# Xiuyu-Li/q-diffusion

Measured on AMD Instinct MI355X. Metric: denoising images/sec (whole node), SD-v1.4 W4A8 512x512 50-step PLMS, higher is better.
Workload: dtype int8xint4->int32 (fp32 residual stream); 1 GPU; sd UNet eval batch 16 per GPU, 51 evals per image batch, W4A8 sm_abit=16 split, hip-graph=on, cross-attention K/V of the run's context prepared once per image batch (2.82 ms, charged as /51 per step); images_per_gpu=8, global_batch=8, context_prepared=True, parallelism=batch-sharded x1, quant-state broadcast 0 B

## Files before the change

q-diffusion_amd/csrc/igemm_dma.hip:

```cpp
#include "common.h"
#include <type_traits>

typedef __attribute__((address_space(3))) void* qd_lds_ptr;

namespace {

__device__ __attribute__((aligned(16))) const int qd_zero16[4] = {0, 0, 0, 0};

struct SegD {
    int c0, clen, kstep0, nsteps_tap;
    const float*  scale;
    const int*    zc;
    const int*    zw;
    const int*    zfill;
    const int8_t* fill16;
};

struct ConvD {
    const int8_t*  x;
    const uint8_t* wt;
    void*          out;
    int32_t*       iout;
    const float*   bias;
    const float*   rowbias;
    const void*    residual;
    long ldx, ldo, ldr, ldrb;
    int B, H, W, Ho, Wo, Cout, kh, kw, stride, pad_t, pad_l;
    int M, taps, nseg, nblk_m, nblk_n, ntiles;
    int vec;
    SegD seg[2];
    const float* oq;
    float oqmin, oqmax;
    int   oqoff;
    int   it_per;
    int   hdH, hdd, hdT, hdTpad, hddpad;
    unsigned hdrcp;
    float oqpre;
    int32_t* hdsum;
    float* gnpart;
    int    gn_nchunk;
    long   gn_ld;
    int    pointwise;
    int    res_f16;
    int    res_period;
    int    ups;
};

enum { O_F32 = 0, O_F16 = 1, O_I32 = 2, O_GEGLU = 3, O_PART = 4, O_HROWS = 5, O_HTR = 6, O_BF16 = 7, O_GEGLU_H = 8 };

template <int N>
__device__ __forceinline__ void wait_vmcnt() {
    asm volatile("s_waitcnt vmcnt(%0)" ::"n"(N) : "memory");
}

__device__ __forceinline__ void glds16(const void* gsrc, unsigned lds_base) {
#ifdef QD_ABL_NODMA
    asm volatile("" ::"v"(gsrc), "s"(lds_base) : "memory");
    return;
#endif
    asm volatile(
        "s_mov_b32 m0, %1\n\t"
        "s_nop 0\n\t"
        "global_load_lds_dwordx4 %0, off"
        :
        : "v"(gsrc), "s"(lds_base)
        : "memory");
}

__device__ __forceinline__ int bytesum16(const v4i& v) {
    int s = __builtin_amdgcn_sdot4(v.x, 0x01010101, 0, false);
    s = __builtin_amdgcn_sdot4(v.y, 0x01010101, s, false);
    s = __builtin_amdgcn_sdot4(v.z, 0x01010101, s, false);
    return __builtin_amdgcn_sdot4(v.w, 0x01010101, s, false);
}

__device__ __forceinline__ unsigned lds_addr(const void* p) {
    return (unsigned)(size_t)(qd_lds_ptr)(p);
}

__device__ __forceinline__ constexpr int crow(int r) { return (r & 3) + 8 * (r >> 2); }

#ifndef QD_MT1_OCC
#define QD_MT1_OCC 2
#endif
template <int MT, int NT, int WM, int WN, int OUT, int WB, int KS = 1>
__host__ __device__ constexpr int igemm_smem_bytes() {
    constexpr bool BF = WB >= 16;
    constexpr int BM = 32 * MT * WM, BN = 32 * NT * WN, NTB = NT * WN;
    constexpr int TB = BF ? 2048 : 256 * WB;
    constexpr int STAGE = BM * 64 + NTB * TB;
    constexpr int TBW = ((OUT == O_F16 || OUT == O_HROWS) && !BF) ? 8192 : 4096;
    constexpr int EPI_BYTES = 4 * KS * TBW + 4 * (32 * NT) * 8;
    constexpr int RING = 3 * KS * STAGE > EPI_BYTES ? 3 * KS * STAGE : EPI_BYTES;
    return RING + (2 + (KS > 1 ? 1 : 0)) * BM * 4 + 4 * BN * 4;
}

template <int MT, int NT, int WM, int WN, bool SPLIT, int OUT, int WB, int KS = 1>
__device__ __forceinline__ void igemm_body(const ConvD& p, unsigned char* smem) {
    static_assert(KS == 1 || (KS == 2 && !SPLIT && WB <= 8 && (OUT == O_F32 || OUT == O_F16 || OUT == O_PART || OUT == O_HROWS || OUT == O_HTR)),
                  "two K-groups: one segment; linear rows, split-K partials or the head-layout epilogues");
    static_assert(WB == 4 || WB == 8 || WB == 16 || WB == 17, "weight bits (16 = bf16 mode, 17 = fp16 mode)");
    constexpr bool BF = WB >= 16;
    constexpr bool FH = WB == 17;
    static_assert(!BF || (!SPLIT && (OUT == O_F32 || OUT == (FH ? O_F16 : O_BF16))), "16-bit float mode: one segment, fp32 rows or rows of the operand type");
    static_assert(WM * WN == 4, "four waves per block");
    constexpr int BM = 32 * MT * WM, BN = 32 * NT * WN, NTB = NT * WN;
    constexpr int TB = BF ? 2048 : 256 * WB;
    constexpr int A_BYTES = BM * 64, B_BYTES = NTB * TB;
    constexpr int STAGE = A_BYTES + B_BYTES;
    constexpr int NA = BM / 64;
    constexpr int NBI = B_BYTES / 1024;
    constexpr int NBW = (NBI + 3) / 4;
    constexpr int PER = NA + NBW;
    constexpr int WCOLS = 32 * NT;

    constexpr int TBW = ((OUT == O_F16 || OUT == O_HROWS) && !BF) ? 8192 : 4096;
    constexpr int EPI_BYTES = 4 * KS * TBW + 4 * WCOLS * 8;
    constexpr int RS = KS * STAGE;
    constexpr int RING = 3 * RS > EPI_BYTES ? 3 * RS : EPI_BYTES;
    static_assert(RING + (2 + (KS > 1 ? 1 : 0)) * BM * 4 + 4 * BN * 4 == igemm_smem_bytes<MT, NT, WM, WN, OUT, WB, KS>(), "igemm_smem_bytes out of step with the body");
    int* sRowB = reinterpret_cast<int*>(smem + RING);
    int* sAsum = sRowB + BM;
    int* sAsum1 = sAsum + BM;
    float* sScale = reinterpret_cast<float*>(sAsum + (KS > 1 ? 2 : 1) * BM);
    int*   sZc    = reinterpret_cast<int*>(sScale + BN);
    int*   sZw    = sZc + BN;
    float* sBias  = reinterpret_cast<float*>(sZw + BN);

    const int lane = threadIdx.x & 63;
    const int wave_all = __builtin_amdgcn_readfirstlane(threadIdx.x >> 6);
    const int kg = KS > 1 ? wave_all >> 2 : 0;
    const int wave = wave_all & 3;
    const int wm = wave / WN, wn = wave % WN;
    const int frow = lane & 31, fhalf = lane >> 5;

    const int nblk    = p.nblk_m * p.nblk_n;
    const int logical = qd_xcd_remap(blockIdx.x, nblk);
    const int mb = logical / p.nblk_n, nb = logical % p.nblk_n;
    const int m0 = mb * BM, n0 = nb * BN;

    const int lr16 = lane >> 2, slot = lane & 3;
    const int a_chunk = (slot ^ ((lr16 >> 2) & 3)) * 16;
    const int8_t* a_org[NA];
    unsigned a_mask[NA];
    int a_hw0[NA];
    bool a_valid[NA];
    const int HoWo = p.Ho * p.Wo;
    if (p.pointwise) {
#pragma unroll
        for (int i = 0; i < NA; ++i) {
            const int r = (wave + 4 * i) * 16 + lr16;
            const int m = m0 + r;
            a_valid[i] = m < p.M;
            const int mm = a_valid[i] ? m : 0;
            a_org[i] = p.x + (long)mm * p.ldx + a_chunk;
            a_mask[i] = a_valid[i] ? 1u : 0u;
            a_hw0[i] = 0;
            if (p.rowbias != nullptr && slot == 0) sRowB[r] = mm / HoWo;
        }
    } else {
#pragma unroll
    for (int i = 0; i < NA; ++i) {
        const int r = (wave + 4 * i) * 16 + lr16;
// ... 819 lines not shown
            int as[16];
            row_terms(rbase, as);
#pragma unroll
            for (int r = 0; r < 16; ++r) {
                const int rl = crow(r) + 4 * fhalf;
                const int I0 = acc[i][j][r] - zc0 - __mul24(zw0, as[r]);
                const int I1 = acc[i][j + 1][r] - zc1 - __mul24(zw1, as[r]);
                float v0, v1;
                if (SPLIT) {
                    v0 = __builtin_fmaf((float)I0, sc0, facc[SPLIT ? i : 0][SPLIT ? j : 0][r]) + bias0;
                    v1 = __builtin_fmaf((float)I1, sc1, facc[SPLIT ? i : 0][SPLIT ? j + 1 : 0][r]) + bias1;
                } else {
                    v0 = __builtin_fmaf((float)I0, sc0, bias0);
                    v1 = __builtin_fmaf((float)I1, sc1, bias1);
                }
                if (rb_tile) { v0 += rbv0; v1 += rbv1; }
                const int pc = frow ^ ((r & 1) << 2);
                tb[rl * 64 + pc] = __float_as_uint(v0);
                tb[rl * 64 + 32 + pc] = __float_as_uint(v1);
            }
            __builtin_amdgcn_sched_barrier(0);
#pragma unroll
            for (int pb = 0; pb < 4; pb += 2) {
            v4i rs[2];
            long mrow[2];
#pragma unroll
            for (int u = 0; u < 2; ++u) {
                const long m = m0 + rbase + (pb + u) * 8 + rr0;
                mrow[u] = m < p.M ? m : m0;
                if (has_res) rs[u] = *reinterpret_cast<const v4i*>(rh + res_row(mrow[u]) * p.ldr + n8c);
            }
#pragma unroll
            for (int u = 0; u < 2; ++u) {
                const int rl = (pb + u) * 8 + rr0;
                const bool mok = m0 + rbase + rl < p.M;
                v4f lo = *reinterpret_cast<const v4f*>(tb + rl * 64 + rd_lo);
                v4f hi = *reinterpret_cast<const v4f*>(tb + rl * 64 + rd_hi);
                if (has_rb && !rb_tile) {
                    const float* src = p.rowbias + (long)sRowB[rbase + rl] * p.ldrb + n8c;
                    lo += *reinterpret_cast<const v4f*>(src);
                    hi += *reinterpret_cast<const v4f*>(src + 4);
                }
                if (has_res) {
                    v4f a, b;
                    qd_h8_to_f(rs[u], a, b);
                    lo += a; hi += b;
                }
                if (mok && nok8) {
                    const v4i pk = {(int)qd_pack2h(lo[0], lo[1]), (int)qd_pack2h(lo[2], lo[3]),
                                    (int)qd_pack2h(hi[0], hi[1]), (int)qd_pack2h(hi[2], hi[3])};
                    *reinterpret_cast<v4i*>(oh + mrow[u] * p.ldo + n8) = pk;
                    if (gn) {
#pragma unroll
                        for (int e = 0; e < 4; ++e) {
                            gs[e] += lo[e]; gq[e] = __builtin_fmaf(lo[e], lo[e], gq[e]);
                            gs[4 + e] += hi[e]; gq[4 + e] = __builtin_fmaf(hi[e], hi[e], gq[4 + e]);
                        }
                    }
                }
            }
            }
        }
        if (gn) {
#pragma unroll
            for (int e = 0; e < 8; ++e) {
#pragma unroll
                for (int sh = 8; sh < 64; sh <<= 1) {
                    gs[e] += __shfl_xor(gs[e], sh);
                    gq[e] += __shfl_xor(gq[e], sh);
                }
            }
            if (lane < 8) {
#pragma unroll
                for (int e = 0; e < 8; ++e) {
                    sGn[(wave * WCOLS + j * 32 + k8 * 8 + e) * 2] = gs[e];
                    sGn[(wave * WCOLS + j * 32 + k8 * 8 + e) * 2 + 1] = gq[e];
                }
            }
        }
        }
    };
    bool lines16 = false;
    if constexpr (H16_OUT && !BF) lines16 = p.vec == 2;
    if (lines16) {
#pragma unroll
        for (int q = 0; q < NT / 2; ++q)
            if (owner(2 * q) == kg) pair(2 * q);
        if constexpr (NT % 2 == 1) {
            if (owner(NT - 1) == kg) single(NT - 1);
        }
    } else {
#pragma unroll
        for (int j = 0; j < NT; ++j)
            if (owner(j) == kg) single(j);
    }
    if (gn) {
        __syncthreads();
        for (int c = threadIdx.x; c < BN; c += 256 * KS)
        if (n0 + c < p.Cout) {
            constexpr int WPC = MT >= 4 ? 1 : 4 / MT;
            const int wnc = c / WCOLS, cw = c - wnc * WCOLS;
#pragma unroll
            for (int ch = 0; ch < BM / 128; ++ch) {
                const int mrow = m0 + ch * 128;
                if (mrow >= p.M) break;
                float ts = 0.f, tq = 0.f;
#pragma unroll
                for (int w = 0; w < WPC; ++w) {
                    const int wv = (ch * WPC + w) * WN + wnc;
                    ts += sGn[(wv * WCOLS + cw) * 2];
                    tq += sGn[(wv * WCOLS + cw) * 2 + 1];
                }
                const int b = mrow / HoWo, chunk = (mrow - b * HoWo) >> 7;
                float* dst = p.gnpart + (((long)b * p.gn_nchunk + chunk) * p.gn_ld + n0 + c) * 2;
                dst[0] = ts;
                dst[1] = tq;
            }
        }
    }
}

template <int MT, int NT, int WM, int WN, bool SPLIT, int OUT, int WB>
__global__ __launch_bounds__(256, (SPLIT || MT * NT > 10) ? 1 : (MT == 1 && NT <= 5 ? QD_MT1_OCC : 2)) void igemm_kernel(const ConvD p) {
    __shared__ __attribute__((aligned(16))) unsigned char smem[igemm_smem_bytes<MT, NT, WM, WN, OUT, WB>()];
    igemm_body<MT, NT, WM, WN, SPLIT, OUT, WB>(p, smem);
}

template <int MT, int NT, int WM, int WN, int OUT, int WB>
__global__ __launch_bounds__(512, 1) void igemm_k2_kernel(const ConvD p) {
    __shared__ __attribute__((aligned(16))) unsigned char smem[igemm_smem_bytes<MT, NT, WM, WN, OUT, WB, 2>()];
    igemm_body<MT, NT, WM, WN, false, OUT, WB, 2>(p, smem);
}

struct ConvG {
    ConvD d[3];
    int   out[3];
};
template <int MT, int NT, int WM, int WN, int WB>
__global__ __launch_bounds__(256, (MT * NT > 10) ? 1 : (MT == 1 && NT <= 5 ? QD_MT1_OCC : 2)) void igemm_heads_group_kernel(const ConvG g) {
    constexpr int SA = igemm_smem_bytes<MT, NT, WM, WN, O_HROWS, WB>(), SB = igemm_smem_bytes<MT, NT, WM, WN, O_HTR, WB>();
    __shared__ __attribute__((aligned(16))) unsigned char smem[SA > SB ? SA : SB];
    const int z = blockIdx.y;
    if (g.out[z] == O_HTR) igemm_body<MT, NT, WM, WN, false, O_HTR, WB>(g.d[z], smem);
    else igemm_body<MT, NT, WM, WN, false, O_HROWS, WB>(g.d[z], smem);
}

__global__ __launch_bounds__(256) void pack_t4_kernel(const float* __restrict__ w, const float* __restrict__ alpha,
                                                      const float* __restrict__ delta, const float* __restrict__ zp,
                                                      int Cout, int Cin_total, int taps, int c0, int clen, int clen_pad,
                                                      int n_levels, uint8_t* __restrict__ wt, int kstep0, int ntiles,
                                                      int nsteps_tap, int32_t* __restrict__ wsum) {
    long gid = (long)blockIdx.x * 256 + threadIdx.x;
    const long total = (long)taps * nsteps_tap * ntiles * 128;
    if (gid >= total) return;
    const int nn = (int)(gid & 31);
    const int kh4 = (int)((gid >> 5) & 3);
    long rest = gid >> 7;
    const int jt = (int)(rest % ntiles);
    rest /= ntiles;
    const int cs = (int)(rest % nsteps_tap);
    const int t = (int)(rest / nsteps_tap);
    const int n = jt * 32 + nn;
    const int cbase = cs * 64 + kh4 * 16;
    int vals[16];
    int sum = 0;
    float d = 1.f, z = 0.f;
    if (n < Cout) { d = delta[n]; z = zp[n]; }
// ... 23 lines not shown
    *reinterpret_cast<uint2*>(wt + (kstep * ntiles + jt) * 1024 + (kh4 * 32 + nn) * 8) = pk;
    if (wsum && sum != 0) atomicAdd(&wsum[n], sum);
}

template <typename TO>
__global__ __launch_bounds__(256) void splitk_finalize_kernel(const int32_t* __restrict__ part, int nsplit, long MN, int Cout, int HoWo,
                                                              const float* __restrict__ scale, const int* __restrict__ zc,
                                                              const int* __restrict__ zw, const int* __restrict__ zfill,
                                                              const float* __restrict__ bias, const float* __restrict__ rowbias, long ldrb,
                                                              const TO* __restrict__ residual, long ldr, TO* __restrict__ out, long ldo) {
    const long e = (long)blockIdx.x * 256 + threadIdx.x;
    if (e >= MN) return;
    const long m = e / Cout;
    const int  n = (int)(e - m * Cout);
    int I = 0;
    for (int s = 0; s < nsplit; ++s) I += part[(long)s * MN + e];
    const int kz = zfill ? zfill[1] : 0;
    I = I - (zc ? zc[n] : 0) + (zw ? zw[n] : 0) * kz;
    float v = __builtin_fmaf((float)I, scale[n], bias ? bias[n] : 0.f);
    if (rowbias) v += rowbias[(m / HoWo) * ldrb + n];
    if constexpr (std::is_same<TO, float>::value) {
        if (residual) v += residual[m * ldr + n];
        out[m * ldo + n] = v;
    } else {
        if (residual) v += __half2float(residual[m * ldr + n]);
        out[m * ldo + n] = __float2half(v);
    }
}

__global__ __launch_bounds__(256) void pack_t8_kernel(const float* __restrict__ w, const float* __restrict__ alpha,
                                                      const float* __restrict__ delta, const float* __restrict__ zp,
                                                      int Cout, int Cin_total, int taps, int c0, int clen,
                                                      int n_levels, uint8_t* __restrict__ wt, int kstep0, int ntiles,
                                                      int nsteps_tap, int32_t* __restrict__ wsum) {
    long gid = (long)blockIdx.x * 256 + threadIdx.x;
    const long total = (long)taps * nsteps_tap * ntiles * 128;
    if (gid >= total) return;
    const int nn = (int)(gid & 31);
    const int kh4 = (int)((gid >> 5) & 3);
    long rest = gid >> 7;
    const int jt = (int)(rest % ntiles);
    rest /= ntiles;
    const int cs = (int)(rest % nsteps_tap);
    const int t = (int)(rest / nsteps_tap);
    const int n = jt * 32 + nn;
    const int cbase = cs * 64 + kh4 * 16;
    int sum = 0;
    float d = 1.f, z = 0.f;
    if (n < Cout) { d = delta[n]; z = zp[n]; }
    v4i pk;
#pragma unroll
    for (int g = 0; g < 4; ++g) {
        unsigned word = 0;
#pragma unroll
        for (int e = 0; e < 4; ++e) {
            const int c = cbase + g * 4 + e;
            int stored = 0;
            if (n < Cout && c < clen) {
                const float wv = w[((long)n * Cin_total + c0 + c) * taps + t];
                float q;
                if (alpha) q = floorf(wv / d) + (alpha[((long)n * clen + c) * taps + t] >= 0.f ? 1.f : 0.f);
                else q = rintf(wv / d);
                q = fminf(fmaxf(q + z, 0.f), (float)(n_levels - 1));
                stored = (int)q - 128;
                sum += stored;
            }
            word |= (unsigned)(stored & 0xff) << (8 * e);
        }
        pk[g] = (int)word;
    }
    const long kstep = kstep0 + (long)t * nsteps_tap + cs;
    *reinterpret_cast<v4i*>(wt + (kstep * ntiles + jt) * 2048 + (kh4 * 32 + nn) * 16) = pk;
    if (wsum && sum != 0) atomicAdd(&wsum[n], sum);
}

#ifdef QD_PROBE_INSTANCE
template __global__ void igemm_kernel<QD_PROBE_INSTANCE>(const ConvD);
}
#else
static int& kgroups_knob() {
    static int v = (getenv("QD_KGROUPS") && atoi(getenv("QD_KGROUPS")) == 0) ? 0 : 1;
    return v;
}

constexpr int kgroups_min_steps() { return 8; }

struct TileId {
    int mt, nt, wm, wn, wb;
    constexpr int bm() const { return 32 * mt * wm; }
    constexpr int bn() const { return 32 * nt * wn; }
    constexpr bool operator==(const TileId& o) const { return mt == o.mt && nt == o.nt && wm == o.wm && wn == o.wn && wb == o.wb; }
};
template <int MT, int NT, int WM, int WN, int WB>
struct Tile { static constexpr TileId id{MT, NT, WM, WN, WB}; };
template <class F>
bool visit_tile(const TileId& id, F f) {
    auto among = [&](auto... t) { return ((decltype(t)::id == id && (f(t), true)) || ...); };
    return among(Tile<1, 5, 4, 1, 4>{}, Tile<1, 7, 4, 1, 4>{}, Tile<1, 4, 4, 1, 4>{}, Tile<1, 2, 4, 1, 4>{}, Tile<2, 5, 4, 1, 4>{}, Tile<2, 4, 4, 1, 4>{}, Tile<2, 5, 2, 2, 4>{},
                 Tile<1, 4, 4, 1, 8>{}, Tile<1, 2, 4, 1, 8>{}, Tile<2, 4, 4, 1, 8>{}, Tile<1, 4, 4, 1, 16>{}, Tile<1, 2, 4, 1, 16>{}, Tile<2, 4, 4, 1, 16>{},
                 Tile<1, 4, 4, 1, 17>{}, Tile<1, 2, 4, 1, 17>{}, Tile<2, 4, 4, 1, 17>{});
}

template <class T>
constexpr bool built(int KS, bool SPLIT, int OUT) {
    constexpr int MT = T::id.mt, NT = T::id.nt, WM = T::id.wm, WB = T::id.wb;
    constexpr bool rows128 = MT == 1 && WM == 4;
    const bool rows = OUT == O_F32 || OUT == O_F16, heads = OUT == O_HROWS || OUT == O_HTR;
    if (WB >= 16) return KS == 1 && !SPLIT && (OUT == O_F32 || OUT == (WB == 16 ? O_BF16 : O_F16));
    if (KS == 2)
        return !SPLIT && (WM == 4 || (MT == 2 && NT == 5)) && (NT == 4 || NT == 5 || NT == 7) && (WB == 4 || NT == 4) &&
               (OUT == O_F32 || (OUT == O_F16 && NT == 5 && MT == 1) || (heads && WB == 4 && NT == 5 && WM == 4) ||
                (OUT == O_PART && rows128 && (WB == 4 ? NT == 5 || NT == 7 : NT == 4)));
    if (SPLIT) return rows && rows128;
    return rows || ((OUT == O_I32 || OUT == O_PART) && rows128) || (OUT == O_GEGLU && NT == 4 && WB == 4 && WM == 4) ||
           (heads && ((WB == 4 && WM == 4) || (WB == 8 && MT == 1 && NT == 4)));
}
constexpr bool group_built(TileId t) { return t.mt == 1 && t.wm == 4 && (t.wb == 4 ? t.nt == 5 || t.nt == 7 || t.nt == 4 : t.wb == 8 && t.nt == 4); }

template <int KS_, bool SPLIT_, int OUT_>
struct Variant { static constexpr int KS = KS_, OUT = OUT_; static constexpr bool SPLIT = SPLIT_; };

struct Launch {
    ConvD  k;
    TileId tile;
    int    out;
    bool   split;
    int    threads, nsplit;
};

TileId choose_tile(int wbits, long M, int N, int out, bool two_seg, bool tall_ok, long Ktot) {
    static const int wide_mink = getenv("QD_WIDE_MINK") ? atoi(getenv("QD_WIDE_MINK")) : 1280;
    static const int wide_minblk = getenv("QD_WIDE_MINBLK") ? atoi(getenv("QD_WIDE_MINBLK")) : 200;
    auto blocks = [&](int bm, int bn) { return ((M + bm - 1) / bm) * ((N + bn - 1) / bn); };
    if (out == O_GEGLU) return {1, 4, 4, 1, wbits};
    const bool rows = out == O_F32 || out == O_F16 || out == O_BF16;
    if (wbits == 4 && N % 320 == 0 && rows && !two_seg && Ktot >= wide_mink && blocks(128, 320) >= wide_minblk) return {2, 5, 2, 2, 4};
    const int nt = wbits < 8 && N % 160 == 0 ? 5 : (wbits < 8 && N % 224 == 0 ? 7 : (N > 64 ? 4 : 2));
    const bool tall = tall_ok && (nt == 4 || nt == 5) && (wbits == 4 || rows) && blocks(256, 32 * nt) >= 256;
    return {tall ? 2 : 1, nt, 4, 1, wbits};
}

int plan_block(Launch* L, TileId tile) {
    ConvD& k = L->k;
    k.nblk_m = (k.M + tile.bm() - 1) / tile.bm();
    k.nblk_n = (k.Cout + tile.bn() - 1) / tile.bn();
    const int ksteps = L->out == O_PART ? k.it_per : k.taps * k.seg[0].nsteps_tap;
    const bool k2 = kgroups_knob() && !L->split && k.nseg == 1 && (long)k.nblk_m * k.nblk_n * L->nsplit <= 256 && ksteps >= kgroups_min_steps();
    bool ok = false;
    L->tile = tile;
    visit_tile(tile, [&](auto t) {
        L->threads = k2 && built<decltype(t)>(2, false, L->out) ? 512 : 256;
        ok = built<decltype(t)>(L->threads / 256, L->split, L->out);
    });
    QD_REQUIRE(ok, "qd_conv2d_%s: unsupported variant split=%d out=%d tile %dx%d", tile.wb >= 16 ? "bf16" : "i8", (int)L->split, L->out, tile.bm(), tile.bn());
    return 0;
}

int launch(const Launch& L, hipStream_t st) {
    const ConvD& k = L.k;
    const dim3 grid(k.nblk_m * k.nblk_n, L.nsplit), block(L.threads);
    bool done = false;
    visit_tile(L.tile, [&](auto t) {
        using T = decltype(t);
        constexpr TileId I = T::id;
        auto variant = [&](auto v) {
            using V = decltype(v);
            if constexpr (built<T>(V::KS, V::SPLIT, V::OUT)) {
                if (L.threads != 256 * V::KS || L.split != V::SPLIT || L.out != V::OUT) return;
                if (k.nblk_m != (k.M + I.bm() - 1) / I.bm() || k.nblk_n != (k.Cout + I.bn() - 1) / I.bn()) return;
                if constexpr (V::KS == 2) hipLaunchKernelGGL((igemm_k2_kernel<I.mt, I.nt, I.wm, I.wn, V::OUT, I.wb>), grid, block, 0, st, k);
                else hipLaunchKernelGGL((igemm_kernel<I.mt, I.nt, I.wm, I.wn, V::SPLIT, V::OUT, I.wb>), grid, block, 0, st, k);
                done = true;
            }
        };
        variant(Variant<2, false, O_F32>{}); variant(Variant<2, false, O_F16>{}); variant(Variant<2, false, O_PART>{}); variant(Variant<2, false, O_HROWS>{});
        variant(Variant<2, false, O_HTR>{}); variant(Variant<1, false, O_F32>{}); variant(Variant<1, false, O_F16>{}); variant(Variant<1, false, O_BF16>{});
        variant(Variant<1, false, O_I32>{}); variant(Variant<1, false, O_PART>{}); variant(Variant<1, false, O_HROWS>{}); variant(Variant<1, false, O_HTR>{});
        variant(Variant<1, false, O_GEGLU>{}); variant(Variant<1, true, O_F32>{}); variant(Variant<1, true, O_F16>{});
    });
    QD_REQUIRE(done, "qd_conv2d: the launch plan names no built kernel (tile %dx%d, %d threads, split=%d out=%d)", L.tile.bm(), L.tile.bn(), L.threads, (int)L.split, L.out);
    return 0;
}

int choose_splitk(const qd_conv_desc* d, int* it_per) {
    *it_per = 0;
    if (d->nseg != 1 || d->epilogue != QD_EPI_LINEAR) return 1;
    if (d->res_period != 0) return 1;
    const long M = (long)d->B * d->Ho * d->Wo;
    const int  N = d->Cout, bn = choose_tile(d->wbits, M, N, O_PART, false, false, 0).bn();
    const long blocks0 = ((M + 127) / 128) * ((N + bn - 1) / bn);
    const int  total = d->kh * d->kw * ((d->seg[0].clen + 63) / 64);
    if (blocks0 > 256) return 1;
    const long mn = M * N;
    const int min_steps = mn <= (1L << 18) ? 2 : (mn <= (3L << 19) ? 4 : 16);
    static const long target = getenv("QD_SPLITK_TARGET") ? atol(getenv("QD_SPLITK_TARGET")) : 256;
    long S = target / blocks0;
    if (S > total / min_steps) S = total / min_steps;
    if (S > 32) S = 32;
    if (S < 2) return 1;
    *it_per = (int)((total + S - 1) / S);
    return (total + *it_per - 1) / *it_per;
}

void fill_geometry(ConvD& k, const qd_conv_desc* d) {
    k.B = d->B; k.H = d->H; k.W = d->W; k.Ho = d->Ho; k.Wo = d->Wo; k.Cout = d->Cout;
    k.kh = d->kh; k.kw = d->kw; k.stride = d->stride; k.pad_t = d->pad_t; k.pad_l = d->pad_l;
    k.M = d->B * d->Ho * d->Wo; k.taps = d->kh * d->kw; k.nseg = d->nseg; k.ntiles = (d->Cout + 31) / 32; k.ups = d->upsample2x ? 1 : 0;
    k.pointwise = k.taps == 1 && d->stride == 1 && d->pad_t == 0 && d->pad_l == 0 && d->H == d->Ho && d->W == d->Wo;
}

int plan(const qd_conv_desc* d, int32_t* iout, bool group_member, Launch* L) {
    QD_REQUIRE(d != nullptr, "qd_conv2d_i8: null descriptor");
    QD_REQUIRE(d->x && d->w && (d->out || iout), "qd_conv2d_i8: null tensor pointer");
    QD_REQUIRE(d->w_tiled, "qd_conv2d_i8: weights must be in the tile order of qd_pack_weights_t4 / _t8 (w_tiled = 1)");
    QD_REQUIRE(d->wbits == 4 || d->wbits == 8, "qd_conv2d_i8: wbits must be 4 or 8 (got %d)", d->wbits);
    QD_REQUIRE(!d->upsample2x || (d->stride == 1 && d->kh * d->kw > 1 && d->H % 2 == 0 && d->W % 2 == 0 && d->pad_t < 8 && d->pad_l < 8),
               "qd_conv2d_i8: upsample2x needs stride 1, more than one tap, even H and W");
    QD_REQUIRE(d->out_dtype == QD_F32 || d->out_dtype == QD_F16, "qd_conv2d_i8: out_dtype must be f32/f16");
    QD_REQUIRE(d->nseg == 1 || d->nseg == 2, "qd_conv2d_i8: nseg must be 1 or 2");
    QD_REQUIRE(d->B > 0 && d->H > 0 && d->W > 0 && d->Ho > 0 && d->Wo > 0 && d->Cout > 0, "qd_conv2d_i8: bad shape");
    QD_REQUIRE(d->kh > 0 && d->kw > 0 && d->stride > 0 && d->kh * d->kw <= 32, "qd_conv2d_i8: bad kernel/stride (at most 32 taps)");
    QD_REQUIRE((long)d->B * d->Ho * d->Wo < (1L << 31), "qd_conv2d_i8: M overflows int32");
    const bool w8 = d->wbits == 8;
    QD_REQUIRE(!w8 || d->epilogue == QD_EPI_LINEAR || ((d->epilogue == QD_EPI_HEADS_I8 || d->epilogue == QD_EPI_HEADS_T_I8) && d->Cout > 64),
               "qd_conv2d_i8: int8 weights take the linear epilogue, or the head-layout epilogues on more than 64 output channels");
    QD_REQUIRE(d->ldx % 16 == 0 && qd_aligned(d->x, 16) && qd_aligned(d->w, 16), "qd_conv2d_i8: x/w must be 16-byte aligned, ldx %% 16 == 0");
    *L = Launch{};
    ConvD& k = L->k;
// ... 172 lines not shown
        pk[gq] = fh ? (int)qd_pack2h(f[0], f[1]) : (int)qd_pack2bf(f[0], f[1]);
    }
    const long kstep = (long)t * nsteps_tap + cs;
    *reinterpret_cast<v4i*>(wt + (kstep * ntiles + jt) * 2048 + (kh4 * 32 + nn) * 16) = pk;
}

}

extern "C" int qd_conv2d_bf16(const qd_conv_desc* d, void* stream) { return run_bf16(d, stream); }

extern "C" int64_t qd_pack_weights_bf16_bytes(int Cout, int taps, int clen_pad) {
    return (int64_t)taps * ((clen_pad + 31) / 32) * ((Cout + 31) / 32) * 2048;
}

extern "C" int qd_pack_weights_h16(const float* w, int Cout, int Cin, int taps, int clen_pad, int wbits, uint8_t* wt, void* stream);
extern "C" int qd_pack_weights_bf16(const float* w, int Cout, int Cin, int taps, int clen_pad, uint8_t* wt, void* stream) {
    return qd_pack_weights_h16(w, Cout, Cin, taps, clen_pad, 16, wt, stream);
}

extern "C" int qd_pack_weights_h16(const float* w, int Cout, int Cin, int taps, int clen_pad, int wbits, uint8_t* wt, void* stream) {
    QD_REQUIRE(wbits == 16 || wbits == 17, "qd_pack_weights_h16: wbits must be 16 (bf16) or 17 (fp16)");
    QD_REQUIRE(w && wt, "qd_pack_weights_bf16: null pointer");
    QD_REQUIRE(Cout > 0 && taps > 0 && Cin > 0, "qd_pack_weights_bf16: bad shape");
    QD_REQUIRE(clen_pad % 8 == 0 && clen_pad >= Cin, "qd_pack_weights_bf16: clen_pad must be a multiple of 8 and >= Cin");
    QD_REQUIRE(qd_aligned(wt, 16), "qd_pack_weights_bf16: wt must be 16-byte aligned");
    const int ntiles = (Cout + 31) / 32, nsteps_tap = (clen_pad + 31) / 32;
    const long total = (long)taps * nsteps_tap * ntiles * 128;
    hipLaunchKernelGGL(pack_bf16_kernel, dim3((unsigned)((total + 255) / 256)), dim3(256), 0, reinterpret_cast<hipStream_t>(stream),
                       w, Cout, Cin, taps, clen_pad, wt, ntiles, nsteps_tap, wbits == 17 ? 1 : 0);
    QD_LAUNCH_CHECK("qd_pack_weights_bf16");
    return 0;
}

extern "C" int64_t qd_conv2d_i8_splitk_ws_bytes(const qd_conv_desc* d) {
    if (!d) return 0;
    int it_per;
    const int S = choose_splitk(d, &it_per);
    return S < 2 ? 0 : (int64_t)S * d->B * d->Ho * d->Wo * d->Cout * 4;
}

int run_group(const qd_conv_desc* const* descs, int n, void* stream) {
    QD_REQUIRE(descs && n >= 1 && n <= 3, "qd_conv2d_i8_group: 1..3 descriptors");
    for (int i = 0; i < n; ++i)
        QD_REQUIRE(!descs[i] || descs[i]->res_period == 0, "qd_conv2d_i8_group: res_period is not supported (head-layout epilogues)");
    if (n == 1) return run(descs[0], nullptr, stream);
    Launch L[3];
    bool ok = true;
    for (int i = 0; i < n; ++i) {
        QD_REQUIRE(descs[i] != nullptr, "qd_conv2d_i8_group: null descriptor");
        if (const int rc = plan(descs[i], nullptr, true, &L[i])) return rc;
        const ConvD &a = L[i].k, &b = L[0].k;
        ok = ok && L[i].nsplit == 1 && !L[i].split && (L[i].out == O_HROWS || L[i].out == O_HTR) && L[i].tile == L[0].tile &&
             a.M == b.M && a.Cout == b.Cout && a.nblk_m == b.nblk_m && a.nblk_n == b.nblk_n;
    }
    bool grouped = false;
    if (ok) visit_tile(L[0].tile, [&](auto t) {
        constexpr TileId I = decltype(t)::id;
        if constexpr (group_built(I)) {
            ConvG g{};
            for (int i = 0; i < n; ++i) { g.d[i] = L[i].k; g.out[i] = L[i].out; }
            dim3 grid(g.d[0].nblk_m * g.d[0].nblk_n, n), block(256);
            hipLaunchKernelGGL((igemm_heads_group_kernel<I.mt, I.nt, I.wm, I.wn, I.wb>), grid, block, 0, reinterpret_cast<hipStream_t>(stream), g);
            grouped = true;
        }
    });
    if (grouped) {
        QD_LAUNCH_CHECK("qd_conv2d_i8_group");
        return 0;
    }
    for (int i = 0; i < n; ++i)
        if (const int rc = run(descs[i], nullptr, stream)) return rc;
    return 0;
}

extern "C" int qd_conv2d_i8_form(const qd_conv_desc* d, int32_t* form4) {
    QD_REQUIRE(form4 != nullptr, "qd_conv2d_i8_form: null form4");
    Launch L;
    if (const int rc = plan(d, nullptr, false, &L)) return rc;
    form4[0] = L.tile.bm(); form4[1] = L.tile.bn(); form4[2] = L.threads; form4[3] = L.nsplit;
    return 0;
}

extern "C" void qd_conv_config(int kgroups) {
    if (kgroups >= 0) kgroups_knob() = kgroups ? 1 : 0;
}
extern "C" int qd_conv2d_i8_group(const qd_conv_desc* const* descs, int n, void* stream) { return run_group(descs, n, stream); }
extern "C" int qd_conv2d_i8(const qd_conv_desc* d, void* stream) { return run(d, nullptr, stream); }
extern "C" int qd_conv2d_i8_acc(const qd_conv_desc* d, int32_t* iout, void* stream) {
    if (!iout) { qd_set_error("qd_conv2d_i8_acc: null iout"); return 1; }
    return run(d, iout, stream);
}

static int pack_weights_tiled(const char* fn, int bits, const float* w, const float* alpha, const float* delta, const float* zp, int Cout, int Cin_total,
                              int taps, int c0, int clen, int clen_pad, int n_levels, uint8_t* wt, int kstep0, int ntiles, int32_t* wsum, void* stream) {
    QD_REQUIRE(w && delta && zp && wt, "%s: null pointer", fn);
    QD_REQUIRE(Cout > 0 && taps > 0 && clen > 0 && c0 >= 0 && c0 + clen <= Cin_total, "%s: bad shape", fn);
    QD_REQUIRE(clen_pad % 16 == 0 && clen_pad >= clen, "%s: clen_pad must be a multiple of 16", fn);
    QD_REQUIRE(n_levels >= 2 && n_levels <= (1 << bits), "%s: n_levels %d does not fit a %s", fn, n_levels, bits == 4 ? "nibble" : "byte");
    QD_REQUIRE(ntiles == (Cout + 31) / 32 && qd_aligned(wt, 16), "%s: bad tile layout", fn);
    const int nsteps_tap = (clen_pad + 63) / 64;
    const long total = (long)taps * nsteps_tap * ntiles * 128;
    const dim3 grid((unsigned)((total + 255) / 256)), block(256);
    hipStream_t st = reinterpret_cast<hipStream_t>(stream);
    if (bits == 4)
        hipLaunchKernelGGL(pack_t4_kernel, grid, block, 0, st, w, alpha, delta, zp, Cout, Cin_total, taps, c0, clen, clen_pad, n_levels, wt, kstep0, ntiles, nsteps_tap, wsum);
    else
        hipLaunchKernelGGL(pack_t8_kernel, grid, block, 0, st, w, alpha, delta, zp, Cout, Cin_total, taps, c0, clen, n_levels, wt, kstep0, ntiles, nsteps_tap, wsum);
    QD_LAUNCH_CHECK(fn);
    return 0;
}
extern "C" int qd_pack_weights_t4(const float* w, const float* alpha, const float* delta, const float* zp, int Cout, int Cin_total, int taps, int c0,
                                  int clen, int clen_pad, int n_levels, uint8_t* wt, int kstep0, int ntiles, int32_t* wsum, void* stream) {
    return pack_weights_tiled("qd_pack_weights_t4", 4, w, alpha, delta, zp, Cout, Cin_total, taps, c0, clen, clen_pad, n_levels, wt, kstep0, ntiles, wsum, stream);
}
extern "C" int qd_pack_weights_t8(const float* w, const float* alpha, const float* delta, const float* zp, int Cout, int Cin_total, int taps, int c0,
                                  int clen, int clen_pad, int n_levels, uint8_t* wt, int kstep0, int ntiles, int32_t* wsum, void* stream) {
    return pack_weights_tiled("qd_pack_weights_t8", 8, w, alpha, delta, zp, Cout, Cin_total, taps, c0, clen, clen_pad, n_levels, wt, kstep0, ntiles, wsum, stream);
}
#endif
```

q-diffusion_amd/qdiff/hip.py:

```python
import ctypes
import os

import torch

_HERE = os.path.dirname(os.path.abspath(__file__))
LIB_PATH = os.environ.get("QDIFF_HIP_LIB") or os.path.join(os.path.dirname(_HERE), "lib", "libqdiff_hip.so")

F32, F16, BF16 = 0, 1, 2
_DT = {torch.float32: F32, torch.float16: F16}


class HipEngineError(RuntimeError):
    pass


class ConvSeg(ctypes.Structure):
    _fields_ = [("c0", ctypes.c_int32), ("clen", ctypes.c_int32), ("kofs", ctypes.c_int32), ("kstep0", ctypes.c_int32),
                ("wzp", ctypes.c_void_p), ("scale", ctypes.c_void_p), ("zc", ctypes.c_void_p), ("zw", ctypes.c_void_p), ("zfill", ctypes.c_void_p),
                ("fill16", ctypes.c_void_p)]


class ConvDesc(ctypes.Structure):
    _fields_ = [("x", ctypes.c_void_p), ("w", ctypes.c_void_p), ("out", ctypes.c_void_p),
                ("bias", ctypes.c_void_p), ("rowbias", ctypes.c_void_p), ("residual", ctypes.c_void_p),
# ... 199 lines not shown

def _qp(t):
    if t is None or t.numel() == 4:
        return t
    if t.numel() != 2:
        raise HipEngineError("qparams must be {delta, zero_point} or the float[4] of make_qparams")
    return make_qparams(t[0], t[1])


def quantize_act(x, B, C, S, strides, qparams, grid, out, ldo, c0=0, clen=None, oc0=0):
    clen = C - c0 if clen is None else clen
    sb, sc, ss = strides
    _check(load().qd_quantize_act(_ptr(x, "x"), _dtype(x), B, C, S, sb, sc, ss, c0, clen, pad16(clen),
                                  _ptr(_qp(qparams), "qparams"), grid.qmin, grid.qmax, grid.off, _ptr(out, "out"), ldo, oc0,
                                  _stream()), "qd_quantize_act")


def pack_weights(w, alpha, delta, zp, Cout, Cin_total, taps, c0, clen, n_levels, mode, wq, ldk, kofs, wsum, codes=None):
    _check(load().qd_pack_weights(_ptr(w), _ptr(alpha), _ptr(delta), _ptr(zp), Cout, Cin_total, taps, c0, clen,
                                  pad16(clen), n_levels, mode, _ptr(wq), ldk, kofs, _ptr(wsum), _ptr(codes), _stream()),
           "qd_pack_weights")


def pack_weights_t4(w, alpha, delta, zp, Cout, Cin_total, taps, c0, clen, n_levels, wt, kstep0, ntiles, wsum):
    _check(load().qd_pack_weights_t4(_ptr(w), _ptr(alpha), _ptr(delta), _ptr(zp), Cout, Cin_total, taps, c0, clen,
                                     pad16(clen), n_levels, _ptr(wt), kstep0, ntiles, _ptr(wsum), _stream()),
           "qd_pack_weights_t4")


def pack_weights_t8(w, alpha, delta, zp, Cout, Cin_total, taps, c0, clen, n_levels, wt, kstep0, ntiles, wsum):
    _check(load().qd_pack_weights_t8(_ptr(w), _ptr(alpha), _ptr(delta), _ptr(zp), Cout, Cin_total, taps, c0, clen,
                                     pad16(clen), n_levels, _ptr(wt), kstep0, ntiles, _ptr(wsum), _stream()),
           "qd_pack_weights_t8")


class ConvCall:
    __slots__ = ("x", "w", "out", "bias", "rowbias", "residual", "ldx", "ldk", "ldo", "ldr", "ld_rowbias",
                 "B", "H", "W", "Ho", "Wo", "Cout", "kh", "kw", "stride", "pad_t", "pad_l", "wbits", "w_tiled", "segs",
                 "epilogue", "oq_params", "oq_grid", "splitk", "heads", "gn_part", "upsample2x", "res_period", "_keep")

    def __init__(self, **kw):
        for k in self.__slots__:
            setattr(self, k, kw.get(k))


_SPLITK_WS = {}


def _splitk_scratch(device, nbytes):
    bufs = _SPLITK_WS.setdefault((device, _stream()), [])
    if not bufs or bufs[-1].numel() < nbytes:
        bufs.append(torch.empty(max(nbytes, 64 << 20), dtype=torch.uint8, device=device))
    return bufs[-1]


def splitk_ws_bytes(c):
    return int(load().qd_conv2d_i8_splitk_ws_bytes(ctypes.byref(_conv_desc(c))))


def _launch_desc(c):
    d = _conv_desc(c)
    if c.w_tiled and c.splitk is not False:
        need = int(load().qd_conv2d_i8_splitk_ws_bytes(ctypes.byref(d)))
        if need:
            ws = _splitk_scratch(c.x.device, need)
            d.splitk_ws, d.splitk_ws_bytes = ws.data_ptr(), ws.numel()
    return d


def conv2d_i8(c, acc_out=None):
    if acc_out is None:
        d = _launch_desc(c)
        _check(load().qd_conv2d_i8(ctypes.byref(d), _stream()), "qd_conv2d_i8")
    else:
        _check(load().qd_conv2d_i8_acc(ctypes.byref(_conv_desc(c)), _ptr(acc_out), _stream()), "qd_conv2d_i8_acc")


def conv2d_i8_form(c):
    form = (ctypes.c_int32 * 4)()
    _check(load().qd_conv2d_i8_form(ctypes.byref(_launch_desc(c)), form), "qd_conv2d_i8_form")
    return tuple(form)


def conv_config(kgroups=-1):
    load().qd_conv_config(int(kgroups))


def conv2d_i8_group(calls):
    descs = [_conv_desc(c) for c in calls]
    arr = (ctypes.POINTER(ConvDesc) * len(descs))(*[ctypes.pointer(d) for d in descs])
    _check(load().qd_conv2d_i8_group(arr, len(descs), _stream()), "qd_conv2d_i8_group")


def _conv_desc(c):
    d = ConvDesc()
    d.x, d.w = _ptr(c.x, "x"), _ptr(c.w, "w")
    d.out = _ptr(c.out, "out")
    d.bias, d.rowbias, d.residual = _ptr(c.bias, "bias"), _ptr(c.rowbias, "rowbias"), _ptr(c.residual, "residual")
    d.ldx, d.ldk, d.ldo = c.ldx, c.ldk, c.ldo or 0
    d.ldr, d.ld_rowbias = c.ldr or 0, c.ld_rowbias or 0
    d.B, d.H, d.W, d.Ho, d.Wo, d.Cout = c.B, c.H, c.W, c.Ho, c.Wo, c.Cout
    d.kh, d.kw, d.stride, d.pad_t, d.pad_l = c.kh, c.kw, c.stride, c.pad_t, c.pad_l
    d.wbits = c.wbits
    d.w_tiled = 1 if c.w_tiled else 0
    d.epilogue = c.epilogue or EPI_LINEAR
    if d.epilogue not in (EPI_LINEAR, EPI_GEGLU_H16):
        c.oq_params = _qp(c.oq_params)
        d.oq_params = _ptr(c.oq_params, "oq_params")
        d.oq_min, d.oq_max, d.oq_off = c.oq_grid.qmin, c.oq_grid.qmax, c.oq_grid.off
        d.out_dtype = _dtype(c.residual) if c.residual is not None else F32
        if d.epilogue in (EPI_HEADS_I8, EPI_HEADS_T_I8):
            hd = c.heads
            d.hd_H, d.hd_d, d.hd_T, d.hd_Tpad, d.hd_dpad = hd["H"], hd["d"], hd["T"], hd["Tpad"], hd["dpad"]
            d.oq_prescale = float(hd["prescale"])
            d.hd_sum = _ptr(hd.get("sum"), "hd_sum")
    elif d.epilogue == EPI_GEGLU_H16:
        d.out_dtype = _H16[c.out.dtype]
    else:
        d.out_dtype = _dtype(c.out) if c.out is not None else F32
    d.gn_part = _ptr(c.gn_part, "gn_part")
    if c.gn_part is not None:
        d.gn_ld = part_ld(c.gn_part)
    d.upsample2x = 1 if c.upsample2x else 0
    d.res_period = int(c.res_period or 0)
    d.nseg = len(c.segs)
    for i, s in enumerate(c.segs):
        g = d.seg[i]
        g.c0, g.clen, g.kofs, g.kstep0 = s["c0"], s["clen"], s["kofs"], s.get("kstep0", 0)
        g.wzp, g.fill16 = _ptr(s.get("wzp"), "wzp"), _ptr(s.get("fill16"), "fill16")
        g.scale, g.zc, g.zw, g.zfill = _ptr(s["scale"], "scale"), _ptr(s.get("zc")), _ptr(s.get("zw")), _ptr(s.get("zfill"))
    return d



def pad8(n):
    return (n + 7) // 8 * 8


def pack_weights_bf16(w, dtype=torch.bfloat16):
    if dtype not in (torch.bfloat16, torch.float16):
        raise HipEngineError("pack_weights_bf16: operand type must be bfloat16 or float16")
    w = w.detach().float().contiguous()
    Cout, Cin = w.shape[0], w.shape[1]
    taps = w[0, 0].numel()
    cpad = pad8(Cin)
    wt = torch.zeros(int(load().qd_pack_weights_bf16_bytes(Cout, taps, cpad)), dtype=torch.uint8, device=w.device)
    _check(load().qd_pack_weights_h16(_ptr(w, "w"), Cout, Cin, taps, cpad, 17 if dtype == torch.float16 else 16, _ptr(wt), _stream()),
           "qd_pack_weights_h16")
    return wt


def conv2d_bf16(x, wt, bias, out, B, H, W, Cin_pad, Cout, k=3, pad=1, residual=None, gn_part=None, upsample2x=False):
    if x.dtype not in (torch.bfloat16, torch.float16) or out.dtype not in (torch.float32, x.dtype):
        raise HipEngineError("conv2d_bf16: x must be bf16 / fp16, out fp32 or x's type")
    if residual is not None and residual.dtype != out.dtype:
        raise HipEngineError("conv2d_bf16: the residual has the type of the output")
    d = ConvDesc()
    d.x, d.w, d.out = _ptr(x, "x"), _ptr(wt, "w"), _ptr(out, "out")
    d.bias, d.residual = _ptr(bias, "bias"), _ptr(residual, "residual")
    d.ldx, d.ldo, d.ldr = x.stride(0), out.stride(0), residual.stride(0) if residual is not None else 0
    d.B, d.H, d.W, d.Ho, d.Wo, d.Cout = B, H, W, H, W, Cout
    d.kh = d.kw = k
    d.stride, d.pad_t, d.pad_l = 1, pad, pad
    d.wbits, d.w_tiled, d.epilogue = (17 if x.dtype == torch.float16 else 16), 1, EPI_LINEAR
    d.out_dtype = BF16 if out.dtype == torch.bfloat16 else F16 if out.dtype == torch.float16 else F32
    d.gn_part = _ptr(gn_part, "gn_part")
    if gn_part is not None:
        d.gn_ld = part_ld(gn_part)
# ... 493 lines not shown
```

Measured before the change: 8.721 images/s.

## Add specialized full-tile epilogue with double-buffered residual/rowbias prefetch

Adds a compile-time specialized epilogue path for integer-GEMM conv tiles that lie fully inside the output bounds. It skips bounds checks and uses 32-bit offset arithmetic, and it software-pipelines the residual or row-bias loads for the next sub-tile into a double buffer while the current one is stored. GroupNorm partial sums are fused into the same path. The path is on by default when strides fit the 32-bit limits, with a knob to fall back to the generic epilogue. The cost is more template instantiations, higher register pressure and larger code size.

```diff
diff --git a/q-diffusion_amd/csrc/igemm_dma.hip b/q-diffusion_amd/csrc/igemm_dma.hip
--- a/q-diffusion_amd/csrc/igemm_dma.hip
+++ b/q-diffusion_amd/csrc/igemm_dma.hip
@@ -44,6 +44,7 @@
     int    res_f16;
     int    res_period;
     int    ups;
+    int    full_ok;
 };
 
 enum { O_F32 = 0, O_F16 = 1, O_I32 = 2, O_GEGLU = 3, O_PART = 4, O_HROWS = 5, O_HTR = 6, O_BF16 = 7, O_GEGLU_H = 8 };
@@ -79,6 +80,9 @@
 }
 
 __device__ __forceinline__ constexpr int crow(int r) { return (r & 3) + 8 * (r >> 2); }
+
+template <int LD_, bool GN_, int JB_, int JE_>
+struct FullTag { static constexpr int LD = LD_, JB = JB_, JE = JE_; static constexpr bool GN = GN_; };
 
 #ifndef QD_MT1_OCC
 #define QD_MT1_OCC 2
@@ -1064,7 +1068,149 @@
     };
     bool lines16 = false;
     if constexpr (H16_OUT && !BF) lines16 = p.vec == 2;
-    if (lines16) {
+    auto full = [&](auto tg) __attribute__((always_inline)) {
+        using TG = decltype(tg);
+        constexpr int LD = TG::LD, JB = TG::JB, JE = TG::JE;
+        constexpr bool GN = TG::GN;
+        constexpr int NTL = (JE - JB) * MT;
+        constexpr bool RAW16 = LD == 1 || OUT == O_F32;
+        using Raw = std::conditional_t<RAW16, v4f, uint2>;
+        constexpr unsigned OSZ = (INT_OUT || OUT == O_F32) ? 4 : 2, LSZ = RAW16 ? 4 : 2;
+        const unsigned ldo_u = INT_OUT ? (unsigned)p.Cout : (unsigned)p.ldo;
+        char* const ob = (INT_OUT ? reinterpret_cast<char*>(oi) : reinterpret_cast<char*>(p.out)) + ((long)(m0 + wrow0) * ldo_u + wcol0) * OSZ;
+        const unsigned olane = ((unsigned)rr0 * ldo_u + c4) * OSZ, ostep = 8u * ldo_u * OSZ;
+        unsigned lofs[LD ? MT : 1][4];
+        const char* lbase = nullptr;
+        if constexpr (LD == 1) {
+            lbase = reinterpret_cast<const char*>(p.rowbias + wcol0);
+#pragma unroll
+            for (int i = 0; i < MT; ++i)
+#pragma unroll
+                for (int ps = 0; ps < 4; ++ps) lofs[i][ps] = ((unsigned)sRowB[wrow0 + i * 32 + ps * 8 + rr0] * (unsigned)p.ldrb + c4) * LSZ;
+        } else if constexpr (LD == 2) {
+            lbase = reinterpret_cast<const char*>(p.residual) + (long)wcol0 * LSZ;
+#pragma unroll
+            for (int i = 0; i < MT; ++i)
+#pragma unroll
+                for (int ps = 0; ps < 4; ++ps) lofs[i][ps] = ((unsigned)res_row((long)m0 + wrow0 + i * 32 + ps * 8 + rr0) * (unsigned)p.ldr + c4) * LSZ;
+        }
+        auto request = [&](const int t, Raw (&b)[4]) __attribute__((always_inline)) {
+            const int j = JB + t / MT, i = t % MT;
+#pragma unroll
+            for (int ps = 0; ps < 4; ++ps) b[ps] = *reinterpret_cast<const Raw*>(lbase + (lofs[i][ps] + (unsigned)j * (32u * LSZ)));
+        };
+        Raw buf[2][4];
+        float gs[4], gq[4];
+#pragma unroll
+        for (int t = 0; t < NTL; ++t) {
+            const int j = JB + t / MT, i = t % MT;
+            const int cl = wn * WCOLS + j * 32 + frow;
+            const float sc = sScale[cl];
+            const int zw_n = sZw[cl];
+            const int zc2 = sZc[cl] - zw_n * kz;
+            const float bias_n = sBias[cl];
+            const int rbase = wrow0 + i * 32;
+            int as[16];
+            if constexpr (!BF) row_terms(rbase, as);
+#pragma unroll
+            for (int r = 0; r < 16; ++r) {
+                const int rl = crow(r) + 4 * fhalf;
+                if constexpr (INT_OUT) {
+                    const int v = OUT == O_PART ? (int)acc[i][j][r] - __mul24(zw_n, as[r])
+                                                : (int)acc[i][j][r] - zc2 - __mul24(zw_n, as[r]);
+                    tb[rl * 32 + frow] = (unsigned)v;
+                } else if constexpr (BF) {
+                    tb[rl * 32 + frow] = __float_as_uint((float)acc[i][j][r] + bias_n);
+                } else {
+                    const int I = acc[i][j][r] - zc2 - __mul24(zw_n, as[r]);
+                    float v;
+                    if (SPLIT) v = __builtin_fmaf((float)I, sc, facc[SPLIT ? i : 0][SPLIT ? j : 0][r]) + bias_n;
+                    else v = __builtin_fmaf((float)I, sc, bias_n);
+                    tb[rl * 32 + frow] = __float_as_uint(v);
+                }
+            }
+            if (GN && i == 0) {
+#pragma unroll
+                for (int e = 0; e < 4; ++e) { gs[e] = 0.f; gq[e] = 0.f; }
+            }
+            if constexpr (LD != 0) {
+                __builtin_amdgcn_sched_barrier(0);
+                if (t == 0) request(0, buf[0]);
+                if (t > 0 && t + 1 < NTL) request(t + 1, buf[(t + 1) & 1]);
+                __builtin_amdgcn_sched_barrier(0);
+            }
+#pragma unroll
+            for (int ps = 0; ps < 4; ++ps) {
+                const int rl = ps * 8 + rr0;
+                char* const ot = ob;
+                const unsigned oo = (unsigned)(i * 4 + ps) * ostep + (olane + (unsigned)j * (32u * OSZ));
+                if constexpr (INT_OUT) {
+                    *reinterpret_cast<v4i*>(ot + oo) = *reinterpret_cast<const v4i*>(tb + rl * 32 + c4);
+                } else {
+                    v4f v = *reinterpret_cast<const v4f*>(tb + rl * 32 + c4);
+                    if constexpr (LD != 0) {
+                        const Raw w = buf[t & 1][ps];
+                        if constexpr (RAW16) v += w;
+                        else if constexpr (B16_OUT) v += qd_ld4bf(&w);
+                        else v += qd_ld4h(reinterpret_cast<const __half*>(&w));
+                    }
+                    if constexpr (OUT == O_F32) *reinterpret_cast<v4f*>(ot + oo) = v;
+                    else if constexpr (B16_OUT) qd_st4bf(ot + oo, v);
+                    else qd_st4h(reinterpret_cast<__half*>(ot + oo), v);
+                    if constexpr (GN) {
+#pragma unroll
+                        for (int e = 0; e < 4; ++e) { gs[e] += v[e]; gq[e] = __builtin_fmaf(v[e], v[e], gq[e]); }
+                    }
+                }
+            }
+            if constexpr (LD != 0) {
+                if (t == 0 && NTL > 1) request(1, buf[1]);
+            }
+            if (GN && i == MT - 1) {
+#pragma unroll
+                for (int e = 0; e < 4; ++e) {
+#pragma unroll
+                    for (int sh = 8; sh < 64; sh <<= 1) {
+                        gs[e] += __shfl_xor(gs[e], sh);
+                        gq[e] += __shfl_xor(gq[e], sh);
+                    }
+                }
+                if (lane < 8) {
+#pragma unroll
+                    for (int e = 0; e < 4; ++e) {
+                        sGn[(wave * WCOLS + j * 32 + c4 + e) * 2] = gs[e];
+                        sGn[(wave * WCOLS + j * 32 + c4 + e) * 2 + 1] = gq[e];
+                    }
+                }
+            }
+        }
+    };
+    constexpr bool FULL_BUILT = !(H16_OUT && !BF && MT == 2) && !(SPLIT && NT == 4);
+    const bool full_tile = FULL_BUILT && vec && !lines16 && p.full_ok && m0 + BM <= p.M && n0 + BN <= p.Cout && !(has_rb && has_res);
+    if (full_tile) {
+        if constexpr (FULL_BUILT) {
+        auto columns = [&](auto jb, auto je) __attribute__((always_inline)) {
+            constexpr int JB = decltype(jb)::value, JE = decltype(je)::value;
+            if constexpr (INT_OUT) {
+                full(FullTag<0, false, JB, JE>{});
+            } else if (gn) {
+                if (has_rb) full(FullTag<1, true, JB, JE>{});
+                else if (has_res) full(FullTag<2, true, JB, JE>{});
+                else full(FullTag<0, true, JB, JE>{});
+            } else {
+                if (has_rb) full(FullTag<1, false, JB, JE>{});
+                else if (has_res) full(FullTag<2, false, JB, JE>{});
+                else full(FullTag<0, false, JB, JE>{});
+            }
+        };
+        if constexpr (KS > 1) {
+            if (kg == 0) columns(std::integral_constant<int, 0>{}, std::integral_constant<int, J0>{});
+            else columns(std::integral_constant<int, J0>{}, std::integral_constant<int, NT>{});
+        } else {
+            columns(std::integral_constant<int, 0>{}, std::integral_constant<int, NT>{});
+        }
+        }
+    } else if (lines16) {
 #pragma unroll
         for (int q = 0; q < NT / 2; ++q)
             if (owner(2 * q) == kg) pair(2 * q);
@@ -1254,6 +1400,10 @@
     static int v = (getenv("QD_KGROUPS") && atoi(getenv("QD_KGROUPS")) == 0) ? 0 : 1;
     return v;
 }
+static int& generic_epilogue_knob() {
+    static int v = 0;
+    return v;
+}
 
 constexpr int kgroups_min_steps() { return 8; }
 
@@ -1316,6 +1466,9 @@
     ConvD& k = L->k;
     k.nblk_m = (k.M + tile.bm() - 1) / tile.bm();
     k.nblk_n = (k.Cout + tile.bn() - 1) / tile.bn();
+    const long ldo = L->out == O_PART || L->out == O_I32 ? k.Cout : k.ldo;
+    k.full_ok = !generic_epilogue_knob() && ldo > 0 && ldo < (1L << 20) && (!k.residual || (k.ldr > 0 && (long)k.M * k.ldr < (1L << 28))) &&
+                (!k.rowbias || (k.ldrb > 0 && (long)k.B * k.ldrb < (1L << 28)));
     const int ksteps = L->out == O_PART ? k.it_per : k.taps * k.seg[0].nsteps_tap;
     const bool k2 = kgroups_knob() && !L->split && k.nseg == 1 && (long)k.nblk_m * k.nblk_n * L->nsplit <= 256 && ksteps >= kgroups_min_steps();
     bool ok = false;
@@ -1654,7 +1807,7 @@
 }
 
 extern "C" void qd_conv_config(int kgroups) {
-    if (kgroups >= 0) kgroups_knob() = kgroups ? 1 : 0;
+    if (kgroups >= 0) { kgroups_knob() = kgroups & 1; generic_epilogue_knob() = (kgroups >> 1) & 1; }
 }
 extern "C" int qd_conv2d_i8_group(const qd_conv_desc* const* descs, int n, void* stream) { return run_group(descs, n, stream); }
 extern "C" int qd_conv2d_i8(const qd_conv_desc* d, void* stream) { return run(d, nullptr, stream); }
diff --git a/q-diffusion_amd/qdiff/hip.py b/q-diffusion_amd/qdiff/hip.py
--- a/q-diffusion_amd/qdiff/hip.py
+++ b/q-diffusion_amd/qdiff/hip.py
@@ -305,8 +305,10 @@
     return tuple(form)
 
 
-def conv_config(kgroups=-1):
-    load().qd_conv_config(int(kgroups))
+def conv_config(kgroups=-1, generic_epilogue=False):
+    if generic_epilogue and int(kgroups) < 0:
+        raise ValueError("conv_config: generic_epilogue is set together with kgroups (0 or 1)")
+    load().qd_conv_config(int(kgroups) if int(kgroups) < 0 else (int(bool(kgroups)) | (2 if generic_epilogue else 0)))
 
 
 def conv2d_i8_group(calls):
```

Result: faster. 9.065 images/s, median of 6 (+4.0%).
